# TheRealOrange/icer_compression

Hardware: AMD Instinct MI355X
Metric: Mpixels/s encode (bit-exact), 4096x4096 gray (higher is better)
Workload: dtype int16

## Files before the change

### icer_compression_amd/csrc/api.hip

```cpp
#include <hip/hip_runtime.h>

#include <algorithm>
#include <atomic>
#include <map>
#include <memory>
#include <mutex>
#include <thread>
#include <sched.h>
#include <time.h>
#include <stdarg.h>
#include <stdio.h>
#include <stdlib.h>
#include <string.h>
#include <string>
#include <vector>

#include "../../include/icer_hip.h"
#include "kernels.hpp"
#include "launch_plan.hpp"
#include "subband_gain.hpp"

using namespace icer;

namespace {
// ... 204 lines not shown
    DevBuf<uint32_t> sub_order, snap_valid;
    DevBuf<Snapshot> snaps;
    DevBuf<SubRecord> sub_recs;
    hipStream_t side_stream = nullptr;
    bool side_stream_borrowed = false;
    hipEvent_t fork[kMaxParts] = {}, join[kMaxParts] = {};
    hipStream_t half_stream = nullptr;
    hipEvent_t part_fork = nullptr, part_join = nullptr;
    hipEvent_t coef_ready = nullptr;
    hipStream_t io_stream = nullptr, copy_stream = nullptr;
    DevBuf<CoderTables> tables;
    DevBuf<uint16_t> in;
    DevBuf<uint8_t> in8;
    DevBuf<uint8_t> out;
    DevBuf<unsigned long long> sizes;
    DevBuf<int32_t> rcs;
    DevBuf<uint64_t> prof;
    DevBuf<unsigned long long> dist;
    DevBuf<uint32_t> fam_weight;
    DevBuf<uint32_t> fam_chan;
    DevBuf<unsigned long long> fam_ll_term;
    hipEvent_t energy_fork[kMaxParts] = {}, energy_join[kMaxParts] = {};
    int dist_frames = 0;
    DevBuf<unsigned long long> curve;
    DevBuf<uint32_t> curve_head;
    DevBuf<BudgetState> budget_state;

    DevBuf<uint64_t> roi_prio;
    DevBuf<uint64_t> roi_keys;
    DevBuf<uint32_t> roi_rank, roi_order;
    DevBuf<uint32_t> roi_bits;

    int *h_flag = nullptr;
    hipEvent_t done = nullptr;
    bool wg_available = true;
    bool sleepy_wait = false;
    struct Pending {
        bool active = false;
        EncodeCall call = {};
    } pend;

    bool timing = false;
    hipEvent_t ev[ICERX_NUM_STAGES + 1] = {};
    double ms[ICERX_NUM_STAGES] = {};
    uint64_t timed_calls = 0;
    bool ev_pending = false;

    int *dwt_ovf(int f0) const { return flags.p + (size_t)f0 * channels; }
    int *mean_ovf(int f0) const { return flags.p + (size_t)max_frames * channels + (size_t)f0 * channels; }
    int *skip(int f0) const { return flags.p + 2 * (size_t)max_frames * channels + f0; }
    int *bound_ovf() const { return flags.p + 2 * (size_t)max_frames * channels + max_frames; }
};

namespace {

struct ClearList {
    static constexpr int kMax = 10;
    uint32_t *p[kMax];
    uint32_t words[kMax];
    int n = 0;
    bool add(void *ptr, size_t bytes)
    {
        if (bytes && (n == kMax || bytes % 4 || bytes / 4 > UINT32_MAX)) return false;
        if (bytes) { p[n] = static_cast<uint32_t *>(ptr); words[n] = (uint32_t)(bytes / 4); n++; }
        return true;
    }
// ... 173 lines not shown
                       b.d_total, e->bound_ovf(), e->budget_state.p);
    hipLaunchKernelGGL(gather_ladder_kernel, dim3(n_units, b.n_frames), dim3(256), 0, c.stream, e->slots.p, e->plan.slot_bytes, e->units.p, n_units,
                       e->unit_bits.p, e->final_off.p, off_pitch, (uint32_t)b.n, c.d_out, c.out_stride, (uint32_t)b.n_frames);
    HIP_TRY(hipGetLastError());
    return 0;
}

int enqueue_part(icerx_encoder *e, const LaunchPlan &lp, int part, bool timed, const EncodeCall &c, bool clear_bound)
{
    const PartPlan &pp = lp.part[part];
    const int f0 = pp.f0, n_frames = pp.n_frames;
    const uint16_t *const d_frames = c.d_frames; uint8_t *const d_out = c.d_out; int32_t *const d_rcs = c.d_rcs;
    unsigned long long *const d_sizes = reinterpret_cast<unsigned long long *>(c.d_sizes);
    const size_t quota = c.quota, out_stride = c.out_stride;
    const hipStream_t st = c.stream; const Ladder *const ladder = c.ladder; const Target *const target = c.target; const Budget *const budget = c.budget;
    const Roi *const roi = c.roi;
    const bool energy = target || budget;
    const bool progressive = lp.progressive, use_wg = lp.use_wg, split = pp.split, hybrid = pp.hybrid;
    const size_t W = e->w, H = e->h, plane = W * H;
    const int C = e->channels, P = n_frames * C;
    const uint32_t n_units = (uint32_t)e->plan.units.size();
    int *dwt_ovf = e->dwt_ovf(f0), *mean_ovf = e->mean_ovf(f0), *skip = e->skip(f0), *bound_ovf = e->bound_ovf();
    int16_t *const coef = e->coef.p + (size_t)f0 * C * plane, *const tmp = e->tmp.p + (size_t)f0 * C * plane;
    unsigned long long *const sums = e->sums.p + (size_t)f0 * C;
    uint16_t *const means = e->means.p + (size_t)f0 * C;
    uint8_t *const sig = e->sig.p + (size_t)f0 * e->plan.sig_bytes;
    uint32_t *const sig_hist = e->sig_hist.p + (size_t)f0 * e->plan.n_families * 16;
    uint8_t *const route_buf = e->route.p + (size_t)f0 * n_units;
    uint32_t *const route_list = e->route_list.p + 2 * (size_t)f0 * n_units,        *const route_ctl = e->route_ctl.p + 4 * (size_t)part;
    uint8_t *const slots = e->slots.p + (size_t)f0 * e->plan.slot_bytes;
    uint32_t *const unit_bits = e->unit_bits.p + (size_t)f0 * n_units, *const done_bytes = e->done_bytes.p + (size_t)f0 * n_units;
    uint64_t *const final_off = e->final_off.p + (size_t)f0 * n_units;
    const size_t sub_entries = e->plan.sub_entries;
    if (split && (e->snaps.ensure((size_t)e->max_frames * sub_entries * kMaxSnaps) || e->snap_valid.ensure((size_t)e->max_frames * sub_entries * kMaxSnaps) ||
                  e->sub_recs.ensure((size_t)e->max_frames * sub_entries))) return ICER_FATAL_ERROR;
    {
        ClearList cl;
        const char *bad = nullptr;
        auto clear = [&](const char *what, void *ptr, size_t bytes) { if (!bad && !cl.add(ptr, bytes)) bad = what; };
        if (f0 == 0 && n_frames == e->max_frames && clear_bound) clear("frame flags", e->flags.p, e->flags.n * sizeof(int));
        else {
            clear("transform flags", dwt_ovf, (size_t)P * sizeof(int)); clear("mean flags", mean_ovf, (size_t)P * sizeof(int)); clear("skip flags", skip, (size_t)n_frames * sizeof(int));
            if (clear_bound) clear("slot bound flag", bound_ovf, sizeof(int));
        }
        clear("LL sums", sums, (size_t)P * sizeof(unsigned long long));
        if (progressive) clear("unit byte counts", done_bytes, (size_t)n_frames * n_units * 4);
        if (hybrid) { clear("chunk histograms", sig_hist, (size_t)n_frames * e->plan.n_families * 16 * sizeof(uint32_t)); clear("route list cursor", route_ctl, 4 * sizeof(uint32_t)); }
        if (split) { clear("snapshot flags", e->snap_valid.p, (size_t)n_frames * sub_entries * kMaxSnaps * sizeof(uint32_t)); clear("sub-range records", e->sub_recs.p, (size_t)n_frames * sub_entries * sizeof(SubRecord)); }
        if (bad) { set_error("enqueue: the clear kernel cannot take the %s range (%d ranges queued)", bad, cl.n); return ICER_FATAL_ERROR; }
        launch_clears(cl, st);
    }
    if (timed && e->timing) HIP_TRY(hipEventRecord(e->ev[0], st));

    size_t cw = W, ch = H;
    launch_dwt(e, d_frames, n_frames, st, e->sample_bits, dwt_ovf, &cw, &ch, coef, tmp);
    if (timed && e->timing) HIP_TRY(hipEventRecord(e->ev[1], st));

    const uint32_t llw = (uint32_t)cw, llh = (uint32_t)ch;
    unsigned sum_blocks = (llw * llh + 255) / 256;
    if (sum_blocks > 64) sum_blocks = 64;
    hipLaunchKernelGGL(ll_sum_kernel, dim3(sum_blocks, P), dim3(256), 0, st, reinterpret_cast<const uint16_t *>(coef),
                       plane, (uint32_t)W, llw, llh, sums, e->sample_bits == 8 ? 0xFFu : 0xFFFFu);
    hipLaunchKernelGGL(ll_mean_kernel, dim3((P + 63) / 64), dim3(64), 0, st, sums, (uint32_t)P, llw * llh,
                       means, mean_ovf, e->sample_bits);
    hipLaunchKernelGGL(frame_status_kernel, dim3((n_frames + 63) / 64), dim3(64), 0, st, dwt_ovf, mean_ovf, C, n_frames, skip);
    hipLaunchKernelGGL(finalize_ll_kernel, dim3((llw + 63u) / 64u, (llh + 3u) / 4u, P), dim3(256), 0, st,
                       reinterpret_cast<uint16_t *>(coef), plane, (uint32_t)W, llw, llh, means, skip, C, e->sample_bits);
    if (timed && e->timing) HIP_TRY(hipEventRecord(e->ev[2], st));
    if (e->coef_ready && f0 == 0) HIP_TRY(hipEventRecord(e->coef_ready, st));

    const int n_planes = e->sample_bits == 8 ? kPlanes8 : kPlanes;
    const size_t ev_frame_bytes = (size_t)n_planes * e->plan.sig_bytes * 64u;
    {
        hipLaunchKernelGGL(family_events_kernel, dim3((unsigned)(e->plan.sig_blocks.size() / 2), n_frames), dim3(256), 0, st,
                           reinterpret_cast<const uint16_t *>(coef), plane, (uint32_t)W, C, e->units.p, e->sig_blocks.p, skip, sig,
                           e->plan.sig_bytes, hybrid ? sig_hist : nullptr, e->plan.n_families,
                           use_wg ? nullptr : e->events.p + (size_t)f0 * ev_frame_bytes, ev_frame_bytes, (uint32_t)n_planes);
    }
    const uint8_t *route = nullptr;
    if (hybrid) {
        hipLaunchKernelGGL(route_units_kernel, dim3((unsigned)((n_units + 255) / 256), n_frames), dim3(256), 0, st, e->units.p, n_units, sig_hist, e->plan.n_families,
                           pp.route_percent, 16u, route_buf, route_list, route_ctl, kNoSplitPercent, (uint32_t)n_frames * n_units, kListHeavyMin);
        route = route_buf;
        HIP_TRY(hipEventRecord(e->fork[part], st));
        HIP_TRY(hipStreamWaitEvent(e->side_stream, e->fork[part], 0));
#define ICER_LAUNCH_LIST(I, NS)                                                                                                          \
        hipLaunchKernelGGL((code_units_list_kernel<I>), dim3(pp.list_grid), dim3(64 * NS::kWgWaves), sizeof(NS::Shared), e->side_stream, \
                           reinterpret_cast<const uint16_t *>(coef), plane, (uint32_t)W, (uint32_t)H, C, e->units.p, n_units,     \
                           e->tables.p, means, skip, slots, e->plan.slot_bytes, unit_bits, sig,                     \
                           e->plan.sig_bytes, route_list, route_ctl, e->prof.p ? e->prof.p + kProfWgsOffset : nullptr, (uint32_t)n_frames * n_units)
        if (pp.list == ListKernel::One) ICER_LAUNCH_LIST(WgOne, wg1); else if (pp.list == ListKernel::Four) ICER_LAUNCH_LIST(WgFour, wg4); else ICER_LAUNCH_LIST(WgSmall, wgs);
#undef ICER_LAUNCH_LIST
        HIP_TRY(hipEventRecord(e->join[part], e->side_stream));
    }
    const uint32_t tgt_planes = (uint32_t)n_planes;
    unsigned long long *const dist = energy ? e->dist.p + (size_t)f0 * e->plan.n_families * (tgt_planes + 1u) : nullptr;
    auto launch_energy = [&](hipStream_t es) -> int {
        HIP_TRY(hipMemsetAsync(dist, 0, (size_t)n_frames * e->plan.n_families * (tgt_planes + 1u) * sizeof(unsigned long long), es));
        hipLaunchKernelGGL(family_energy_kernel, dim3((unsigned)(e->plan.sig_blocks.size() / 2), n_frames), dim3(64 * kEnergyWaves), 0, es,
                           reinterpret_cast<const uint16_t *>(coef), plane, (uint32_t)W, C, e->units.p, e->sig_blocks.p, dist, e->plan.n_families, tgt_planes);
// ... 40 lines not shown
                           sig, e->plan.sig_bytes)
        if (pp.window == WindowKernel::Four) ICER_LAUNCH_WG(WgFour, wg4); else ICER_LAUNCH_WG(WgFull, wg);
#undef ICER_LAUNCH_WG
    }
    if (timed && e->timing) HIP_TRY(hipEventRecord(e->ev[3], st));

    if (energy) {
        if (e->side_stream) HIP_TRY(hipStreamWaitEvent(st, e->energy_join[part], 0));
        else if (launch_energy(st)) return ICER_FATAL_ERROR;
    }
    if (budget) {
        const size_t curve_pitch = (size_t)n_units + 1u;
        hipLaunchKernelGGL(curve_kernel, dim3(n_frames), dim3(64), 0, st, unit_bits, n_units, (uint64_t)quota, skip, e->units.p, dist, e->fam_weight.p,
                           e->plan.n_families, tgt_planes, e->fam_ll_term.p, e->fam_chan.p, means, C, e->curve.p + (size_t)f0 * curve_pitch,
                           e->curve.p + ((size_t)e->max_frames + f0) * curve_pitch, e->curve_head.p + (size_t)f0 * kCurveHeadWords);
        if (lp.n_parts == 1 && enqueue_budget_tail(e, c)) return ICER_FATAL_ERROR;
    } else if (target) {
        const size_t off_pitch = (size_t)e->max_frames * n_units;
        hipLaunchKernelGGL(scan_target_kernel, dim3(n_frames, target->n), dim3(64), 0, st, unit_bits, e->final_order.p, n_units, target->thresholds,
                           (uint64_t)quota, skip, final_off, off_pitch, d_sizes, d_rcs, (uint32_t)target->pitch, e->units.p, bound_ovf, dist,
                           e->fam_weight.p, e->plan.n_families, tgt_planes, e->fam_ll_term.p, e->fam_chan.p, means, C, target->d_reached + f0, target->d_dist + f0, target->d_equiv + f0);
        hipLaunchKernelGGL(gather_ladder_kernel, dim3(n_units, n_frames), dim3(256), 0, st, slots, e->plan.slot_bytes,
                           e->units.p, n_units, unit_bits, final_off, off_pitch, (uint32_t)target->n, d_out, out_stride, (uint32_t)target->pitch);
    } else if (roi) {
        const size_t off_pitch = (size_t)e->max_frames * n_units;
        uint32_t *const rank = e->roi_rank.p + (size_t)f0 * n_units, *const order = e->roi_order.p + (size_t)f0 * n_units;
        hipLaunchKernelGGL(roi_rank_kernel, dim3(n_frames), dim3(64 * kRoiWaves), 0, st, e->units.p, n_units, e->roi_prio.p, roi->d_rois + 4 * (size_t)f0,
                           roi->shift, (uint32_t)W, (uint32_t)H, e->roi_keys.p + (size_t)f0 * n_units, rank, order, roi->d_foreground + f0);
        hipLaunchKernelGGL(scan_roi_kernel, dim3(n_frames, roi->n), dim3(64), 0, st, unit_bits, e->final_order.p, n_units, roi->quotas, skip, rank, order,
                           e->roi_bits.p + (size_t)f0 * n_units, final_off, off_pitch, d_sizes, d_rcs, roi->d_kept + f0, (uint32_t)roi->pitch, e->units.p, bound_ovf);
        hipLaunchKernelGGL(gather_ladder_kernel, dim3(n_units, n_frames), dim3(256), 0, st, slots, e->plan.slot_bytes,
                           e->units.p, n_units, unit_bits, final_off, off_pitch, (uint32_t)roi->n, d_out, out_stride, (uint32_t)roi->pitch);
    } else if (!ladder || ladder->n == 1) {
        hipLaunchKernelGGL(scan_kernel, dim3(n_frames), dim3(64), 0, st, unit_bits, e->final_order.p, n_units,
                           (uint64_t)quota, skip, final_off, d_sizes, d_rcs, e->units.p, bound_ovf);
        hipLaunchKernelGGL(gather_kernel, dim3(n_units, n_frames), dim3(256), 0, st, slots, e->plan.slot_bytes,
                           e->units.p, n_units, unit_bits, final_off, d_out, out_stride);
    } else {
        const size_t off_pitch = (size_t)e->max_frames * n_units;
        hipLaunchKernelGGL(scan_ladder_kernel, dim3(n_frames, ladder->n), dim3(64), 0, st, unit_bits, e->final_order.p, n_units,
                           ladder->quotas, skip, final_off, off_pitch, d_sizes, d_rcs, (uint32_t)ladder->pitch, e->units.p, bound_ovf);
        hipLaunchKernelGGL(gather_ladder_kernel, dim3(n_units, n_frames), dim3(256), 0, st, slots, e->plan.slot_bytes,
                           e->units.p, n_units, unit_bits, final_off, off_pitch, (uint32_t)ladder->n, d_out, out_stride, (uint32_t)ladder->pitch);
    }
    if (timed && e->timing) {
        HIP_TRY(hipEventRecord(e->ev[4], st));
        e->ev_pending = true;
    }
    HIP_TRY(hipGetLastError());
    return 0;
}

int enqueue(icerx_encoder *e, const EncodeCall &c, bool overlap_ok)
{
    const hipStream_t st = c.stream;
    const CoderState cs{e->wg_available, e->wg_once, e->half_stream != nullptr};
    const LaunchPlan &lp = e->last_plan = plan_launch(launch_shape(e), e->tuning, cs, c.n_frames, c.quota, overlap_ok, c.roi != nullptr);
    if (lp.n_parts == 1) return enqueue_part(e, lp, 0, true, c, true);
    HIP_TRY(hipMemsetAsync(e->bound_ovf(), 0, sizeof(int), st));
    HIP_TRY(hipEventRecord(e->part_fork, st));
    HIP_TRY(hipStreamWaitEvent(e->half_stream, e->part_fork, 0));
    if (e->timing) { HIP_TRY(hipEventRecord(e->ev[0], st)); HIP_TRY(hipEventRecord(e->ev[1], st)); HIP_TRY(hipEventRecord(e->ev[2], st)); }
    for (int k = 0; k < lp.n_parts; k++) {
        EncodeCall pc = c.frames(lp.part[k].f0, lp.part[k].n_frames, (size_t)e->channels * e->w * e->h);
        pc.stream = (k & 1) ? e->half_stream : st;
        if (int rc = enqueue_part(e, lp, k, false, pc, false)) return rc;
    }
    HIP_TRY(hipEventRecord(e->part_join, e->half_stream));
// ... 68 lines not shown
#define CREATE_TRY(expr) do { hipError_t e_ = (expr); if (e_ != hipSuccess) { set_error("%s failed: %s (%s:%d)", #expr, hipGetErrorString(e_), __FILE__, __LINE__); icerx_encoder_destroy(e); return ICER_FATAL_ERROR; } } while (0)
    CREATE_TRY(hipSetDevice(device));
    const size_t P = (size_t)max_frames * channels, plane = w * h, n_units = e->plan.units.size();
    if (e->coef.ensure(P * plane) || e->tmp.ensure(P * plane) || e->sums.ensure(P) || e->means.ensure(P) ||
        e->flags.ensure(2 * P + 2 * max_frames + 1) || e->unit_bits.ensure((size_t)max_frames * n_units) ||
        e->done_bytes.ensure((size_t)max_frames * n_units) || e->route.ensure((size_t)max_frames * n_units) || e->route_list.ensure(2 * (size_t)max_frames * n_units) || e->route_ctl.ensure(4 * kMaxParts) || e->sig.ensure((size_t)max_frames * e->plan.sig_bytes + 64) || e->sig_hist.ensure((size_t)max_frames * e->plan.n_families * 16 + 16) ||
        e->final_off.ensure((size_t)max_frames * n_units) || e->tables.ensure(1) || e->sizes.ensure(max_frames) ||
        e->rcs.ensure(max_frames)) {
        icerx_encoder_destroy(e);
        return ICER_FATAL_ERROR;
    }
    if (e->tuning.coder != 2 && e->events.ensure((size_t)max_frames * (size_t)(sample_bits == 8 ? kPlanes8 : kPlanes) * e->plan.sig_bytes * 64u + 64)) {
        icerx_encoder_destroy(e);
        return ICER_FATAL_ERROR;
    }
    CREATE_TRY(hipMemcpy(e->tables.p, &g_tables, sizeof g_tables, hipMemcpyHostToDevice));
    if (hipFuncSetAttribute(reinterpret_cast<const void *>(code_units_wg_kernel<WgFull>), hipFuncAttributeMaxDynamicSharedMemorySize, (int)sizeof(wg::Shared)) != hipSuccess ||
        hipFuncSetAttribute(reinterpret_cast<const void *>(code_units_wg_kernel<WgFour>), hipFuncAttributeMaxDynamicSharedMemorySize, (int)sizeof(wg4::Shared)) != hipSuccess ||
        hipFuncSetAttribute(reinterpret_cast<const void *>(code_units_list_kernel<WgSmall>), hipFuncAttributeMaxDynamicSharedMemorySize, (int)sizeof(wgs::Shared)) != hipSuccess ||
        hipFuncSetAttribute(reinterpret_cast<const void *>(code_units_list_kernel<WgOne>), hipFuncAttributeMaxDynamicSharedMemorySize, (int)sizeof(wg1::Shared)) != hipSuccess ||
        hipFuncSetAttribute(reinterpret_cast<const void *>(code_units_list_kernel<WgFour>), hipFuncAttributeMaxDynamicSharedMemorySize, (int)sizeof(wg4::Shared)) != hipSuccess ||
        create_side_stream(&e->side_stream) != hipSuccess ||
        create_part_events(e) != hipSuccess) {
        (void)hipGetLastError();
        e->wg_available = false;
        if (e->tuning.coder == 2) { set_error("ICER_HIP_CODER=wg, but this device does not grant the workgroup coder its LDS block"); icerx_encoder_destroy(e); return ICER_FATAL_ERROR; }
        fprintf(stderr, "libicer_hip: the workgroup coder is not available on this device; the wave pipeline codes everything\n");
    }
#ifdef ICER_PHASE_TIMERS
    if (e->prof.ensure(kProfWords)) { icerx_encoder_destroy(e); return ICER_FATAL_ERROR; }
    CREATE_TRY(hipMemset(e->prof.p, 0, kProfWords * sizeof(uint64_t)));
#endif
    for (auto &ev : e->ev) CREATE_TRY(hipEventCreate(&ev));
    CREATE_TRY(hipHostMalloc((void **)&e->h_flag, (2 + kMaxParts) * sizeof(int), hipHostMallocDefault));
    CREATE_TRY(hipEventCreateWithFlags(&e->done, hipEventDisableTiming));
#undef CREATE_TRY
    *out = e;
    return 0;
}

void icerx_encoder_destroy(icerx_encoder *e)
{
    if (!e) return;
    (void)hipSetDevice(e->device);
    e->coef.release(); e->tmp.release(); e->sums.release(); e->means.release(); e->flags.release();
    e->units.release(); e->work_order.release(); e->final_order.release(); e->unit_bits.release(); e->done_bytes.release(); e->sig.release(); e->events.release(); e->sig_hist.release(); e->sig_blocks.release(); e->route.release(); e->route_list.release(); e->route_ctl.release();
    e->final_off.release(); e->slots.release(); e->tables.release(); e->in.release(); e->in8.release(); e->out.release();
    e->sizes.release(); e->rcs.release(); e->prof.release();
    e->subs.release(); e->sub_order.release(); e->snap_valid.release(); e->snaps.release(); e->sub_recs.release();
    e->dist.release(); e->fam_weight.release(); e->fam_chan.release(); e->fam_ll_term.release();
    e->curve.release(); e->curve_head.release(); e->budget_state.release();
    e->roi_prio.release(); e->roi_keys.release(); e->roi_rank.release(); e->roi_order.release(); e->roi_bits.release();
    for (auto &ev : e->energy_fork) if (ev) (void)hipEventDestroy(ev);
    for (auto &ev : e->energy_join) if (ev) (void)hipEventDestroy(ev);
    for (auto &ev : e->ev) if (ev) (void)hipEventDestroy(ev);
    if (e->done) (void)hipEventDestroy(e->done);
    for (auto &ev : e->fork) if (ev) (void)hipEventDestroy(ev);
    for (auto &ev : e->join) if (ev) (void)hipEventDestroy(ev);
    if (e->part_fork) (void)hipEventDestroy(e->part_fork);
    if (e->part_join) (void)hipEventDestroy(e->part_join);
    if (e->half_stream) (void)hipStreamDestroy(e->half_stream);
    if (e->side_stream && !e->side_stream_borrowed) (void)hipStreamDestroy(e->side_stream);
    if (e->coef_ready) (void)hipEventDestroy(e->coef_ready);
    if (e->io_stream) (void)hipStreamDestroy(e->io_stream);
    if (e->copy_stream) (void)hipStreamDestroy(e->copy_stream);
    if (e->h_flag) (void)hipHostFree(e->h_flag);
    delete e;
// ... 9 lines not shown
    std::vector<uint32_t> bits((size_t)n_frames * n_units);
    if (!n_units || hipMemcpy(bits.data(), e->unit_bits.p, bits.size() * sizeof(uint32_t), hipMemcpyDeviceToHost) != hipSuccess) return;
    int shown = 0;
    for (size_t i = 0; i < bits.size() && shown < 4; i++) {
        if (bits[i] != kUnitFailed) continue;
        const size_t frame = i / n_units, ui = i % n_units;
        const UnitDesc &u = e->plan.units[ui];
        uint32_t dbg[kFailWords] = {0};
        if (u.cap_words >= kFailWords)
            (void)hipMemcpy(dbg, e->slots.p + frame * e->plan.slot_bytes + u.slot_off + kHeaderBytes, sizeof dbg, hipMemcpyDeviceToHost);
        fprintf(stderr, "libicer_hip: time-out in frame %zu unit %zu (chan %u level %u subband %u lsb %u seg %u, %u x %u)", frame, ui,
                (unsigned)u.chan, (unsigned)u.level, (unsigned)u.subband, (unsigned)u.lsb, (unsigned)u.seg, (unsigned)u.w, (unsigned)u.h);
        if (dbg[0] == kFailMagic)
            fprintf(stderr, ": wave %u gave up at coder_core.hpp:%u; chunks %u, done pixel/count/compact/merge %u/%u/%u/%u, ring alloc/popped "
                    "%u/%u, hold seq/ack %u/%u, generation %u (last exact %u), bitpos %u, flushed words %u, drain_exit %u",
                    dbg[1] >> 16, dbg[1] & 0xFFFFu, dbg[2], dbg[3], dbg[4], dbg[5], dbg[6], dbg[7], dbg[8], dbg[9], dbg[10], dbg[11],
                    dbg[12], dbg[13], dbg[14], dbg[15]);
        fprintf(stderr, "\n");
        shown++;
    }
}

size_t row_stride(const icerx_encoder *e, size_t quota) { return std::min(quota, e->plan.slot_bytes) + 4; }
bool stride_admissible(const icerx_encoder *e, size_t out_stride, size_t quota) { return out_stride >= quota || out_stride >= e->plan.slot_bytes; }

int encode_begin(icerx_encoder *e, const EncodeCall &c, int *flag, hipEvent_t done)
{
    if (upload_units(e, c.quota, c.stream)) return ICER_FATAL_ERROR;
    if (e->slots.ensure((size_t)e->max_frames * e->plan.slot_bytes)) return ICER_FATAL_ERROR;
    if (!stride_admissible(e, c.out_stride, c.quota)) {
        set_error("icerx_encode_device: out_stride %zu smaller than the byte quota %zu", c.out_stride, c.quota);
        return ICER_INVALID_INPUT;
    }
    if (enqueue(e, c, c.overlap_ok && flag == e->h_flag)) return ICER_FATAL_ERROR;
    HIP_TRY(hipMemcpyAsync(flag, e->bound_ovf(), sizeof(int), hipMemcpyDeviceToHost, c.stream));
    for (int k = 0; k < e->last_plan.n_parts; k++)
        if (e->last_plan.part[k].hybrid) HIP_TRY(hipMemcpyAsync(flag + 1 + k, e->route_ctl.p + 4 * k, sizeof(int), hipMemcpyDeviceToHost, c.stream));
    HIP_TRY(hipEventRecord(done, c.stream));
    return 0;
}

static int wait_event(hipEvent_t ev, bool sleepy)
{
    for (uint32_t polls = 0;; polls++) {
        const hipError_t q = hipEventQuery(ev);
        if (q == hipSuccess) return 0;
        if (q != hipErrorNotReady) { set_error("hipEventQuery failed: %s", hipGetErrorString(q)); return ICER_FATAL_ERROR; }
        if (sleepy && polls > 64u) { const struct timespec ts = {0, 50000}; nanosleep(&ts, nullptr); }
        else cpu_relax();
    }
}

static int encode_verdict(icerx_encoder *e, int n_frames, const int *flag)
{
    const int ovf = flag[0];
    if (!ovf) {
        bool routed = false;
        for (int k = 0; k < e->last_plan.n_parts; k++) if (e->last_plan.part[k].hybrid) { routed = true; e->n_routed_units += (uint64_t)(uint32_t)flag[1 + k]; }
        if (routed) e->n_routed_launches++;
        return 0;
    }
    if (ovf & 2) {
        report_timeouts(e, n_frames);
        e->n_timeouts++; g_stats[0]++;
        if (e->wg_once || !e->wg_available) {
            e->wg_once = false;
            set_error(e->wg_available ? "a coding unit timed out in the workgroup-window coder"
                                      : "a coding unit timed out and the barrier-only coder is not available on this device");
            return ICER_FATAL_ERROR;
        }
// ... 977 lines not shown
```

### icer_compression_amd/csrc/dwt_tile.hpp

```cpp
#pragma once
#include <stdint.h>

#if defined(__HIPCC__)
#define DWT_HD __host__ __device__ __forceinline__
#else
#define DWT_HD static inline
#endif
#include "icer_tables.hpp"

#if defined(__HIPCC__)
#define DWT_UNROLL _Pragma("unroll")
#else
#define DWT_UNROLL
#endif

namespace icer {

constexpr int kTileKX = 64, kTileKY = 16;
constexpr int kWinW = 2 * kTileKX + 8, kWinH = 2 * kTileKY + 8;
constexpr int kWinPX = kWinW / 2, kWinPY = kWinH / 2;
constexpr int kTileThreads = 256;

struct DwtTileShared {
    union {
// ... 13 lines not shown
    const int16_t *src;
    uint32_t src_stride;
    int cw, ch;
    int16_t *coef;
    uint32_t coef_stride;
    int16_t *ll;
    uint32_t ll_stride;
    FilterTaps f;
    int32_t lim;
    int sm;
};

DWT_HD int16_t to_coder_word(int16_t v, int sm)
{
    if (sm == 16) {
        const uint16_t mask = (uint16_t)(v >> 15);
        return (int16_t)((((uint16_t)v + mask) ^ mask) | ((uint16_t)v & 0x8000u));
    }
    if (sm == 8) {
        const int8_t v8 = (int8_t)v;
        const uint8_t m8 = (uint8_t)(v8 >> 7);
        const uint8_t w8 = (uint8_t)((((uint8_t)v8 + m8) ^ m8) | ((uint8_t)v8 & 0x80u));
        return (int16_t)(uint16_t)(((w8 & 0x80u) << 8) | (w8 & 0x7Fu));
    }
    return v;
}

DWT_HD int tile_x0(int tx) { return 2 * tx * kTileKX - 4; }
DWT_HD int tile_y0(int ty) { return 2 * ty * kTileKY - 4; }

DWT_HD void dwt_tile_load(DwtTileShared &sh, const DwtStageArgs &a, int tx, int ty, int t)
{
    const int x0 = tile_x0(tx), y0 = tile_y0(ty);
    const bool words = ((a.src_stride & 1u) == 0u) && ((reinterpret_cast<uintptr_t>(a.src) & 3u) == 0u);
    for (int i = t; i < kWinH * kWinPX; i += kTileThreads) {
        const int r = i / kWinPX, p = i - r * kWinPX;
        const int gx = x0 + 2 * p, gy = y0 + r;
        int16_t v0 = 0, v1 = 0;
        if (gy >= 0 && gy < a.ch && gx + 1 >= 0 && gx < a.cw) {
            const int16_t *q = a.src + (size_t)gy * a.src_stride + gx;
            if (words && gx >= 0 && gx + 1 < a.cw) {
                const uint32_t w = *reinterpret_cast<const uint32_t *>(q);
                v0 = (int16_t)(w & 0xFFFFu); v1 = (int16_t)(w >> 16);
            } else {
                if (gx >= 0) v0 = q[0];
                if (gx + 1 < a.cw) v1 = q[1];
            }
        }
        sh.win[r][2 * p] = v0; sh.win[r][2 * p + 1] = v1;
    }
}

DWT_HD bool dwt_pair_step1(int32_t a, int32_t b, int n, int k, int32_t lim, int16_t *low, int16_t *dif)
{
    const int nh = n >> 1;
    bool ovf = false;
    if (k < nh) {
        const int32_t v = (a + b) >> 1, d = a - b;
        ovf = v < -lim - 1 || v > lim || d < -lim - 1 || d > lim;
        *low = (int16_t)v; *dif = (int16_t)d;
    } else { *low = (int16_t)a; *dif = 0; }
    return ovf;
}

template <class Lo, class Di>
DWT_HD bool dwt_pair_step2(const Lo &LO, const Di &DI, int n, int k, int am1, int a0, int a1, int be, int32_t lim, int16_t *high)
{
    const int nl = (n + 1) >> 1, nh = n >> 1;
    const bool odd = (n & 1) != 0;
    const auto clampi = [nl](int j) { return j < 0 ? 0 : (j > nl - 1 ? nl - 1 : j); };
    const int32_t l0 = LO(clampi(k - 2)), l1 = LO(clampi(k - 1)), l2 = LO(k), l3 = LO(clampi(k + 1));
    const int32_t r_km1 = (int16_t)(l0 - l1), r_k = (int16_t)(l1 - l2), r_kp1 = (int16_t)(l2 - l3);
    const int32_t dk = DI(k);
    const int32_t dn = (k + 1 < nh) ? (int32_t)DI(k + 1) : 0;
    int32_t sub;
    if (k == 0) sub = r_kp1 >> 2;
    else if (k == 1 && am1 != 0) {
        const int32_t x = (odd && nl == 3) ? 0 : dk;
        sub = (2 * r_k + 3 * r_kp1 - 2 * x + 4) >> 3;
    } else if (!odd && k == nh - 1) sub = r_k >> 2;
    else {
        const int32_t rm = (k >= 2) ? r_km1 : 1;
// ... 222 lines not shown
```

### icer_compression_amd/csrc/kernels.hpp

```cpp
#pragma once
#include <hip/hip_runtime.h>

#include "assemble_core.hpp"
#include "assemble_ladder.hpp"
#include "roi_core.hpp"
#include "coder_core.hpp"
#include "distortion_core.hpp"
#include "budget_core.hpp"
#include "coder_wg.hpp"
#include "coder_wg_small.hpp"
#include "dwt_tile.hpp"
#include "events.hpp"
#include "plan.hpp"

namespace icer {

__global__ void __launch_bounds__(kTileThreads)
dwt_tile_kernel(DwtStageArgs a, size_t src_plane, size_t coef_plane, size_t ll_plane, int *__restrict__ ovf)
{
    __shared__ union { DwtTileShared gen; DwtFastShared fast; } u;
    a.src += blockIdx.z * src_plane;
    a.coef += blockIdx.z * coef_plane;
    a.ll += blockIdx.z * ll_plane;
    const int tx = blockIdx.x, ty = blockIdx.y, t = threadIdx.x;
// ... 26 lines not shown
              unsigned long long *__restrict__ sums, uint32_t mask)
{
    const uint16_t *p = coef + blockIdx.y * plane;
    const uint32_t n = llw * llh;
    unsigned long long acc = 0;
    for (uint32_t i = blockIdx.x * 256 + threadIdx.x; i < n; i += gridDim.x * 256) {
        const uint32_t r = i / llw, c = i - r * llw;
        acc += p[(size_t)r * stride + c] & mask;
    }
    for (int o = 32; o > 0; o >>= 1) acc += __shfl_down(acc, o);
    if ((threadIdx.x & 63) == 0 && acc) atomicAdd(&sums[blockIdx.y], acc);
}

__global__ void ll_mean_kernel(const unsigned long long *__restrict__ sums, uint32_t n_planes, uint32_t ll_count,
                               uint16_t *__restrict__ means, int *__restrict__ mean_ovf, int sample_bits)
{
    const uint32_t p = blockIdx.x * blockDim.x + threadIdx.x;
    if (p >= n_planes) return;
    const uint16_t m = sample_bits == 8 ? (uint16_t)(uint8_t)(sums[p] / ll_count) : (uint16_t)(sums[p] / ll_count);
    means[p] = m;
    mean_ovf[p] = m > (sample_bits == 8 ? 127 : 32767) ? 1 : 0;
}

__global__ void __launch_bounds__(256)
finalize_ll_kernel(uint16_t *__restrict__ coef, size_t plane, uint32_t w, uint32_t llw, uint32_t llh,
                   const uint16_t *__restrict__ means, const int *__restrict__ frame_skip, int channels, int sample_bits)
{
    const uint32_t c = blockIdx.x * 64 + (threadIdx.x & 63), r = blockIdx.y * 4 + (threadIdx.x >> 6);
    if (c >= llw || r >= llh) return;
    if (frame_skip[blockIdx.z / channels]) return;
    uint16_t *q = coef + blockIdx.z * plane + (size_t)r * w + c;
    const int16_t v = (int16_t)((int16_t)*q - (int16_t)means[blockIdx.z]);
    *q = (uint16_t)to_coder_word(v, sample_bits);
}

struct SplitLaunch {
    const SubDesc *subs = nullptr;
    const uint32_t *launch = nullptr;
    uint32_t n_subs = 0;
    uint32_t entries = 0;
    Snapshot *snaps = nullptr;
    uint32_t *snap_valid = nullptr;
    SubRecord *recs = nullptr;
};

constexpr uint8_t kRoutePipeline = 0, kRouteWindows = 1, kRouteNoSplit = 2;

template <int WAVES, int OCC, int LDS_PAD>
__global__ void __launch_bounds__(64 * WAVES, OCC)
code_units_kernel(const uint16_t *__restrict__ coef, size_t plane, uint32_t img_w, uint32_t img_h, int channels,
                  const UnitDesc *__restrict__ units, const uint32_t *__restrict__ work_order, uint32_t n_units,
                  const CoderTables *__restrict__ tables, const uint16_t *__restrict__ means,
                  const int *__restrict__ frame_skip, uint8_t *__restrict__ slots,
                  size_t slot_frame_stride, uint32_t *__restrict__ unit_bits, uint64_t *__restrict__ timers,
                  uint32_t *__restrict__ done_bytes, uint64_t early_quota, const uint8_t *__restrict__ route, SplitLaunch sp, uint32_t n_frames_1d,
                  const uint8_t *__restrict__ ev, size_t ev_frame_stride, const uint8_t *__restrict__ sig, size_t sig_frame_stride,
                  uint32_t fail_inject)
{
    __shared__ CoderShared s;
    if constexpr (LDS_PAD > 0) {
        __shared__ uint32_t lds_pad[LDS_PAD / 4];
        if (early_quota == ~0ull) lds_pad[threadIdx.x] = 1u;
    }
    uint32_t frame = blockIdx.y, lpos = blockIdx.x;
    if (gridDim.y == 1u && n_frames_1d > 1u) {
        position_major(blockIdx.x, n_units + sp.n_subs, n_frames_1d, &frame, &lpos);
// ... 453 lines not shown
                       size_t slot_frame_stride, uint32_t *__restrict__ unit_bits,
                       const uint8_t *__restrict__ sig, size_t sig_frame_stride,
                       const uint32_t *__restrict__ list, uint32_t *__restrict__ list_ctl, uint64_t *__restrict__ timers, uint32_t list_cap)
{
    extern __shared__ __attribute__((aligned(16))) unsigned char wg_lds[];
    typename I::Shared &s = *reinterpret_cast<typename I::Shared *>(wg_lds);
    __shared__ uint32_t next_entry;
    wg_shared_tables<I>(s, tables);
    const WgLaunch L{coef, plane, img_w, img_h, channels, units, n_units, means, frame_skip, slots, slot_frame_stride, unit_bits, timers,
                     nullptr, 0ull, sig, sig_frame_stride};
    const uint32_t count = list_ctl[0], n_heavy = list_ctl[2];
    for (;;) {
        __syncthreads();
        if (threadIdx.x == 0) next_entry = atomicAdd(&list_ctl[1], 1u);
        __syncthreads();
        const uint32_t at = next_entry;
        if (at >= count) break;
        const uint32_t e = at < n_heavy ? list[list_cap + at] : list[at - n_heavy];
#ifdef ICER_PHASE_TIMERS
        const uint64_t t_start = wall_clock64();
#endif
        wg_code_one_unit<I>(s, L, e / n_units, e % n_units);
#ifdef ICER_PHASE_TIMERS
        if (timers && threadIdx.x == 0 && at < (uint32_t)kListTrace && e < n_units) {
            const UnitDesc &ud = units[e];
            uint64_t *tr = timers + 9 * 32 + 4 * at;
            tr[0] = t_start; tr[1] = wall_clock64(); tr[2] = blockIdx.x | ((uint64_t)e << 32);
            tr[3] = (uint64_t)ud.lsb | ((uint64_t)ud.level << 8) | ((uint64_t)ud.subband << 16) | ((uint64_t)ud.seg << 24) | ((uint64_t)((ud.w * ud.h + 63u) / 64u) << 32);
        }
#endif
    }
}

__global__ void __launch_bounds__(64)
scan_kernel(const uint32_t *__restrict__ unit_bits, const uint32_t *__restrict__ final_order, uint32_t n_units,
            uint64_t quota, const int *__restrict__ frame_skip, uint64_t *__restrict__ final_off,
            unsigned long long *__restrict__ sizes, int32_t *__restrict__ rcs, const UnitDesc *__restrict__ units,
            int *__restrict__ bound_overflow)
{
    const uint32_t frame = blockIdx.x;
    uint64_t *foff = final_off + (size_t)frame * n_units;
    if (frame_skip[frame]) {
        for (uint32_t i = threadIdx.x; i < n_units; i += 64) foff[i] = ~0ull;
        if (threadIdx.x == 0) { sizes[frame] = 0; rcs[frame] = kIntegerOverflow; }
        return;
    }
    const uint32_t *bits = unit_bits + (size_t)frame * n_units;
    {
        int failed = 0;
        for (uint32_t i = threadIdx.x; i < n_units; i += 64) failed |= bits[i] == kUnitFailed;
        if (__ballot(failed)) {
            for (uint32_t i = threadIdx.x; i < n_units; i += 64) foff[i] = ~0ull;
            if (threadIdx.x == 0) { sizes[frame] = 0; rcs[frame] = kFatalError; atomicOr(bound_overflow, 2); }
            return;
        }
    }
    uint32_t kept;
    uint64_t used;
    const int rc = scan_frame_wave(bits, final_order, n_units, quota, foff, &kept, &used);
    if (kept < n_units && threadIdx.x == 0 && bits[kept] == kUnitTooBig && units[kept].cap_is_bound)
        atomicOr(bound_overflow, 1);
    if (threadIdx.x == 0) { sizes[frame] = used; rcs[frame] = rc; }
}

__global__ void __launch_bounds__(256)
gather_kernel(const uint8_t *__restrict__ slots, size_t slot_frame_stride, const UnitDesc *__restrict__ units,
              uint32_t n_units, const uint32_t *__restrict__ unit_bits, const uint64_t *__restrict__ final_off,
              uint8_t *__restrict__ out, size_t out_stride)
{
    const uint32_t frame = blockIdx.y, ui = blockIdx.x;
    const uint64_t off = final_off[(size_t)frame * n_units + ui];
    if (off == ~0ull) return;
    const uint32_t len = kHeaderBytes + ((unit_bits[(size_t)frame * n_units + ui] + 7u) >> 3);
    const uint8_t *src = slots + (size_t)frame * slot_frame_stride + units[ui].slot_off;
    uint8_t *dst = out + (size_t)frame * out_stride + off;
    const uint32_t mis = (uint32_t)((4u - ((uintptr_t)dst & 3u)) & 3u);
    const uint32_t head = mis < len ? mis : len;
    if (threadIdx.x < head) dst[threadIdx.x] = src[threadIdx.x];
    const uint32_t body_words = (len - head) >> 2;
    const uint32_t *sw = reinterpret_cast<const uint32_t *>(src);
    uint32_t *dw = reinterpret_cast<uint32_t *>(dst + head);
    const uint32_t shift = head * 8;
    for (uint32_t i = threadIdx.x; i < body_words; i += 256) {
        const uint32_t lo = sw[i];
        uint32_t v = lo;
        if (shift) v = (lo >> shift) | (sw[i + 1] << (32 - shift));
        dw[i] = v;
    }
    const uint32_t done = head + body_words * 4;
    if (threadIdx.x < len - done) dst[done + threadIdx.x] = src[done + threadIdx.x];
}


__global__ void __launch_bounds__(64)
scan_ladder_kernel(const uint32_t *__restrict__ unit_bits, const uint32_t *__restrict__ final_order, uint32_t n_units,
// ... 156 lines not shown
```

Baseline: 3407.

## Fuse LL mean stages, parallelize scan, write verdict via mapped memory, batch DWT loads

For small LL bands, one block-per-plane kernel now replaces the four-kernel sum/mean/status/finalize sequence, and the LL-sums clear is dropped. The one-wave scan kernel becomes a 256-thread block scan with a cut search. The verdict words are written straight into mapped coherent host memory instead of being fetched with extra device-to-host memcpys. The DWT tile load is restructured to issue all loads before the LDS stores. This trims launch and copy overhead but adds a system-scope write, whose visibility ordering and bit-exactness carry risk.

```diff
diff --git a/icer_compression_amd/csrc/api.hip b/icer_compression_amd/csrc/api.hip
--- a/icer_compression_amd/csrc/api.hip
+++ b/icer_compression_amd/csrc/api.hip
@@ -260,6 +260,9 @@
     DevBuf<uint32_t> roi_bits;
 
     int *h_flag = nullptr;
+    int *d_flag = nullptr;
+    bool verdict_wanted = false;
+    bool verdict_written = false;
     hipEvent_t done = nullptr;
     bool wg_available = true;
     bool sleepy_wait = false;
@@ -499,6 +502,9 @@
     uint32_t *const unit_bits = e->unit_bits.p + (size_t)f0 * n_units, *const done_bytes = e->done_bytes.p + (size_t)f0 * n_units;
     uint64_t *const final_off = e->final_off.p + (size_t)f0 * n_units;
     const size_t sub_entries = e->plan.sub_entries;
+    size_t ll_w = W, ll_h = H;
+    for (int s = 0; s < e->stages; s++) { ll_w = (ll_w + 1) / 2; ll_h = (ll_h + 1) / 2; }
+    const bool ll_fused = P <= (int)kLlFusedMaxPlanes && ll_w * ll_h <= kLlFusedMaxSamples;
     if (split && (e->snaps.ensure((size_t)e->max_frames * sub_entries * kMaxSnaps) || e->snap_valid.ensure((size_t)e->max_frames * sub_entries * kMaxSnaps) ||
                   e->sub_recs.ensure((size_t)e->max_frames * sub_entries))) return ICER_FATAL_ERROR;
     {
@@ -510,7 +516,7 @@
             clear("transform flags", dwt_ovf, (size_t)P * sizeof(int)); clear("mean flags", mean_ovf, (size_t)P * sizeof(int)); clear("skip flags", skip, (size_t)n_frames * sizeof(int));
             if (clear_bound) clear("slot bound flag", bound_ovf, sizeof(int));
         }
-        clear("LL sums", sums, (size_t)P * sizeof(unsigned long long));
+        if (!ll_fused) clear("LL sums", sums, (size_t)P * sizeof(unsigned long long));
         if (progressive) clear("unit byte counts", done_bytes, (size_t)n_frames * n_units * 4);
         if (hybrid) { clear("chunk histograms", sig_hist, (size_t)n_frames * e->plan.n_families * 16 * sizeof(uint32_t)); clear("route list cursor", route_ctl, 4 * sizeof(uint32_t)); }
         if (split) { clear("snapshot flags", e->snap_valid.p, (size_t)n_frames * sub_entries * kMaxSnaps * sizeof(uint32_t)); clear("sub-range records", e->sub_recs.p, (size_t)n_frames * sub_entries * sizeof(SubRecord)); }
@@ -524,15 +530,21 @@
     if (timed && e->timing) HIP_TRY(hipEventRecord(e->ev[1], st));
 
     const uint32_t llw = (uint32_t)cw, llh = (uint32_t)ch;
-    unsigned sum_blocks = (llw * llh + 255) / 256;
-    if (sum_blocks > 64) sum_blocks = 64;
-    hipLaunchKernelGGL(ll_sum_kernel, dim3(sum_blocks, P), dim3(256), 0, st, reinterpret_cast<const uint16_t *>(coef),
-                       plane, (uint32_t)W, llw, llh, sums, e->sample_bits == 8 ? 0xFFu : 0xFFFFu);
-    hipLaunchKernelGGL(ll_mean_kernel, dim3((P + 63) / 64), dim3(64), 0, st, sums, (uint32_t)P, llw * llh,
-                       means, mean_ovf, e->sample_bits);
-    hipLaunchKernelGGL(frame_status_kernel, dim3((n_frames + 63) / 64), dim3(64), 0, st, dwt_ovf, mean_ovf, C, n_frames, skip);
-    hipLaunchKernelGGL(finalize_ll_kernel, dim3((llw + 63u) / 64u, (llh + 3u) / 4u, P), dim3(256), 0, st,
-                       reinterpret_cast<uint16_t *>(coef), plane, (uint32_t)W, llw, llh, means, skip, C, e->sample_bits);
+    const uint32_t ll_mask = e->sample_bits == 8 ? 0xFFu : 0xFFFFu;
+    if (ll_fused) {
+        hipLaunchKernelGGL(ll_fused_kernel, dim3(P), dim3(kLlFusedThreads), 0, st, reinterpret_cast<uint16_t *>(coef), plane, (uint32_t)W, llw, llh,
+                           ll_mask, C, e->sample_bits, dwt_ovf, means, mean_ovf, skip);
+    } else {
+        unsigned sum_blocks = (llw * llh + 255) / 256;
+        if (sum_blocks > 64) sum_blocks = 64;
+        hipLaunchKernelGGL(ll_sum_kernel, dim3(sum_blocks, P), dim3(256), 0, st, reinterpret_cast<const uint16_t *>(coef),
+                           plane, (uint32_t)W, llw, llh, sums, ll_mask);
+        hipLaunchKernelGGL(ll_mean_kernel, dim3((P + 63) / 64), dim3(64), 0, st, sums, (uint32_t)P, llw * llh,
+                           means, mean_ovf, e->sample_bits);
+        hipLaunchKernelGGL(frame_status_kernel, dim3((n_frames + 63) / 64), dim3(64), 0, st, dwt_ovf, mean_ovf, C, n_frames, skip);
+        hipLaunchKernelGGL(finalize_ll_kernel, dim3((llw + 63u) / 64u, (llh + 3u) / 4u, P), dim3(256), 0, st,
+                           reinterpret_cast<uint16_t *>(coef), plane, (uint32_t)W, llw, llh, means, skip, C, e->sample_bits);
+    }
     if (timed && e->timing) HIP_TRY(hipEventRecord(e->ev[2], st));
     if (e->coef_ready && f0 == 0) HIP_TRY(hipEventRecord(e->coef_ready, st));
 
@@ -639,8 +651,13 @@
         hipLaunchKernelGGL(gather_ladder_kernel, dim3(n_units, n_frames), dim3(256), 0, st, slots, e->plan.slot_bytes,
                            e->units.p, n_units, unit_bits, final_off, off_pitch, (uint32_t)roi->n, d_out, out_stride, (uint32_t)roi->pitch);
     } else if (!ladder || ladder->n == 1) {
-        hipLaunchKernelGGL(scan_kernel, dim3(n_frames), dim3(64), 0, st, unit_bits, e->final_order.p, n_units,
-                           (uint64_t)quota, skip, final_off, d_sizes, d_rcs, e->units.p, bound_ovf);
+        VerdictWords verdict;
+        if (e->verdict_wanted && lp.n_parts == 1 && n_frames == 1) {
+            verdict.host = e->d_flag; verdict.route_ctl = hybrid ? route_ctl : nullptr;
+            e->verdict_written = true;
+        }
+        hipLaunchKernelGGL(scan_kernel, dim3(n_frames), dim3(kScanThreads), 0, st, unit_bits, e->final_order.p, n_units,
+                           (uint64_t)quota, skip, final_off, d_sizes, d_rcs, e->units.p, bound_ovf, verdict);
         hipLaunchKernelGGL(gather_kernel, dim3(n_units, n_frames), dim3(256), 0, st, slots, e->plan.slot_bytes,
                            e->units.p, n_units, unit_bits, final_off, d_out, out_stride);
     } else {
@@ -775,7 +792,14 @@
     CREATE_TRY(hipMemset(e->prof.p, 0, kProfWords * sizeof(uint64_t)));
 #endif
     for (auto &ev : e->ev) CREATE_TRY(hipEventCreate(&ev));
-    CREATE_TRY(hipHostMalloc((void **)&e->h_flag, (2 + kMaxParts) * sizeof(int), hipHostMallocDefault));
+    const char *const verdict_mode = getenv("ICER_HIP_VERDICT");
+    if ((verdict_mode && !strcmp(verdict_mode, "copy")) ||
+        hipHostMalloc((void **)&e->h_flag, (2 + kMaxParts) * sizeof(int), hipHostMallocMapped | hipHostMallocCoherent) != hipSuccess ||
+        hipHostGetDevicePointer((void **)&e->d_flag, e->h_flag, 0) != hipSuccess) {
+        (void)hipGetLastError();
+        e->d_flag = nullptr;
+        if (!e->h_flag) CREATE_TRY(hipHostMalloc((void **)&e->h_flag, (2 + kMaxParts) * sizeof(int), hipHostMallocDefault));
+    }
     CREATE_TRY(hipEventCreateWithFlags(&e->done, hipEventDisableTiming));
 #undef CREATE_TRY
     *out = e;
@@ -851,10 +875,14 @@
         set_error("icerx_encode_device: out_stride %zu smaller than the byte quota %zu", c.out_stride, c.quota);
         return ICER_INVALID_INPUT;
     }
+    e->verdict_wanted = flag == e->h_flag && e->d_flag;
+    e->verdict_written = false;
     if (enqueue(e, c, c.overlap_ok && flag == e->h_flag)) return ICER_FATAL_ERROR;
-    HIP_TRY(hipMemcpyAsync(flag, e->bound_ovf(), sizeof(int), hipMemcpyDeviceToHost, c.stream));
-    for (int k = 0; k < e->last_plan.n_parts; k++)
-        if (e->last_plan.part[k].hybrid) HIP_TRY(hipMemcpyAsync(flag + 1 + k, e->route_ctl.p + 4 * k, sizeof(int), hipMemcpyDeviceToHost, c.stream));
+    if (!e->verdict_written) {
+        HIP_TRY(hipMemcpyAsync(flag, e->bound_ovf(), sizeof(int), hipMemcpyDeviceToHost, c.stream));
+        for (int k = 0; k < e->last_plan.n_parts; k++)
+            if (e->last_plan.part[k].hybrid) HIP_TRY(hipMemcpyAsync(flag + 1 + k, e->route_ctl.p + 4 * k, sizeof(int), hipMemcpyDeviceToHost, c.stream));
+    }
     HIP_TRY(hipEventRecord(done, c.stream));
     return 0;
 }
diff --git a/icer_compression_amd/csrc/dwt_tile.hpp b/icer_compression_amd/csrc/dwt_tile.hpp
--- a/icer_compression_amd/csrc/dwt_tile.hpp
+++ b/icer_compression_amd/csrc/dwt_tile.hpp
@@ -69,22 +69,26 @@
 DWT_HD void dwt_tile_load(DwtTileShared &sh, const DwtStageArgs &a, int tx, int ty, int t)
 {
     const int x0 = tile_x0(tx), y0 = tile_y0(ty);
-    const bool words = ((a.src_stride & 1u) == 0u) && ((reinterpret_cast<uintptr_t>(a.src) & 3u) == 0u);
-    for (int i = t; i < kWinH * kWinPX; i += kTileThreads) {
+    constexpr int kIters = (kWinH * kWinPX + kTileThreads - 1) / kTileThreads;
+    int16_t v0[kIters], v1[kIters];
+    DWT_UNROLL
+    for (int k = 0; k < kIters; k++) {
+        const int i = t + k * kTileThreads;
         const int r = i / kWinPX, p = i - r * kWinPX;
         const int gx = x0 + 2 * p, gy = y0 + r;
-        int16_t v0 = 0, v1 = 0;
-        if (gy >= 0 && gy < a.ch && gx + 1 >= 0 && gx < a.cw) {
-            const int16_t *q = a.src + (size_t)gy * a.src_stride + gx;
-            if (words && gx >= 0 && gx + 1 < a.cw) {
-                const uint32_t w = *reinterpret_cast<const uint32_t *>(q);
-                v0 = (int16_t)(w & 0xFFFFu); v1 = (int16_t)(w >> 16);
-            } else {
-                if (gx >= 0) v0 = q[0];
-                if (gx + 1 < a.cw) v1 = q[1];
-            }
-        }
-        sh.win[r][2 * p] = v0; sh.win[r][2 * p + 1] = v1;
+        const bool row_in = i < kWinH * kWinPX && gy >= 0 && gy < a.ch;
+        const bool in0 = row_in && gx >= 0 && gx < a.cw, in1 = row_in && gx + 1 >= 0 && gx + 1 < a.cw;
+        const size_t at0 = in0 ? (size_t)gy * a.src_stride + (size_t)gx : 0u, at1 = in1 ? (size_t)gy * a.src_stride + (size_t)(gx + 1) : 0u;
+        const int16_t s0 = a.src[at0], s1 = a.src[at1];
+        v0[k] = in0 ? s0 : (int16_t)0;
+        v1[k] = in1 ? s1 : (int16_t)0;
+    }
+    DWT_UNROLL
+    for (int k = 0; k < kIters; k++) {
+        const int i = t + k * kTileThreads;
+        if (i >= kWinH * kWinPX) break;
+        const int r = i / kWinPX, p = i - r * kWinPX;
+        sh.win[r][2 * p] = v0[k]; sh.win[r][2 * p + 1] = v1[k];
     }
 }
 
diff --git a/icer_compression_amd/csrc/kernels.hpp b/icer_compression_amd/csrc/kernels.hpp
--- a/icer_compression_amd/csrc/kernels.hpp
+++ b/icer_compression_amd/csrc/kernels.hpp
@@ -82,6 +82,66 @@
     uint16_t *q = coef + blockIdx.z * plane + (size_t)r * w + c;
     const int16_t v = (int16_t)((int16_t)*q - (int16_t)means[blockIdx.z]);
     *q = (uint16_t)to_coder_word(v, sample_bits);
+}
+
+constexpr uint32_t kLlFusedThreads = 1024, kLlFusedMaxSamples = 1u << 16, kLlFusedMaxPlanes = 4, kLlFusedBatch = 8;
+__global__ void __launch_bounds__(kLlFusedThreads)
+ll_fused_kernel(uint16_t *__restrict__ coef, size_t plane, uint32_t stride, uint32_t llw, uint32_t llh, uint32_t mask, int channels,
+                int sample_bits, const int *__restrict__ dwt_ovf, uint16_t *__restrict__ means, int *__restrict__ mean_ovf,
+                int *__restrict__ frame_skip)
+{
+    __shared__ unsigned long long wave_sum[kLlFusedThreads / 64];
+    const uint32_t p = blockIdx.x, frame = p / (uint32_t)channels, n = llw * llh;
+    int skip = 0;
+    uint16_t mean = 0;
+    for (uint32_t q = frame * (uint32_t)channels; q < (frame + 1u) * (uint32_t)channels; q++) {
+        const uint16_t *src = coef + q * plane;
+        unsigned long long acc = 0;
+        for (uint32_t base = threadIdx.x; base < n; base += kLlFusedBatch * kLlFusedThreads) {
+            uint32_t v[kLlFusedBatch];
+#pragma unroll
+            for (uint32_t k = 0; k < kLlFusedBatch; k++) {
+                const uint32_t i = base + k * kLlFusedThreads, ii = i < n ? i : 0u;
+                const uint32_t r = ii / llw, c = ii - r * llw;
+                const uint32_t x = src[(size_t)r * stride + c];
+                v[k] = i < n ? x & mask : 0u;
+            }
+#pragma unroll
+            for (uint32_t k = 0; k < kLlFusedBatch; k++) acc += v[k];
+        }
+        for (int o = 32; o > 0; o >>= 1) acc += __shfl_down(acc, o);
+        if ((threadIdx.x & 63) == 0) wave_sum[threadIdx.x >> 6] = acc;
+        __syncthreads();
+        unsigned long long sum = 0;
+        for (uint32_t w = 0; w < kLlFusedThreads / 64; w++) sum += wave_sum[w];
+        __syncthreads();
+        const uint16_t m = sample_bits == 8 ? (uint16_t)(uint8_t)(sum / n) : (uint16_t)(sum / n);
+        const int ovf = m > (sample_bits == 8 ? 127 : 32767) ? 1 : 0;
+        skip |= dwt_ovf[q] | ovf;
+        if (q == p) {
+            mean = m;
+            if (threadIdx.x == 0) { means[p] = m; mean_ovf[p] = ovf; }
+        }
+    }
+    if (threadIdx.x == 0 && p == frame * (uint32_t)channels) frame_skip[frame] = skip;
+    if (skip) return;
+    uint16_t *dst = coef + p * plane;
+    for (uint32_t base = threadIdx.x; base < n; base += kLlFusedBatch * kLlFusedThreads) {
+        uint16_t v[kLlFusedBatch];
+        size_t at[kLlFusedBatch];
+#pragma unroll
+        for (uint32_t k = 0; k < kLlFusedBatch; k++) {
+            const uint32_t i = base + k * kLlFusedThreads, ii = i < n ? i : 0u;
+            const uint32_t r = ii / llw, c = ii - r * llw;
+            at[k] = (size_t)r * stride + c;
+            v[k] = dst[at[k]];
+        }
+#pragma unroll
+        for (uint32_t k = 0; k < kLlFusedBatch; k++) {
+            if (base + k * kLlFusedThreads >= n) break;
+            dst[at[k]] = (uint16_t)to_coder_word((int16_t)((int16_t)v[k] - (int16_t)mean), sample_bits);
+        }
+    }
 }
 
 struct SplitLaunch {
@@ -601,35 +661,100 @@
     }
 }
 
-__global__ void __launch_bounds__(64)
+struct VerdictWords {
+    int *host = nullptr;
+    const uint32_t *route_ctl = nullptr;
+};
+
+constexpr uint32_t kScanThreads = 256;
+
+__device__ inline uint64_t scan_block_exclusive(uint64_t v, uint64_t *wave_tot, uint64_t *total)
+{
+    const uint32_t lane = threadIdx.x & 63u, wv = threadIdx.x >> 6;
+    uint64_t inc = v;
+    for (uint32_t o = 1; o < 64u; o <<= 1) {
+        const uint64_t t = __shfl_up((unsigned long long)inc, o);
+        if (lane >= o) inc += t;
+    }
+    if (lane == 63u) wave_tot[wv] = inc;
+    __syncthreads();
+    uint64_t base = 0, tot = 0;
+    for (uint32_t w = 0; w < kScanThreads / 64u; w++) {
+        const uint64_t x = wave_tot[w];
+        if (w < wv) base += x;
+        tot += x;
+    }
+    __syncthreads();
+    *total = tot;
+    return base + inc - v;
+}
+
+__global__ void __launch_bounds__(kScanThreads)
 scan_kernel(const uint32_t *__restrict__ unit_bits, const uint32_t *__restrict__ final_order, uint32_t n_units,
             uint64_t quota, const int *__restrict__ frame_skip, uint64_t *__restrict__ final_off,
             unsigned long long *__restrict__ sizes, int32_t *__restrict__ rcs, const UnitDesc *__restrict__ units,
-            int *__restrict__ bound_overflow)
-{
+            int *__restrict__ bound_overflow, VerdictWords verdict)
+{
+    __shared__ uint64_t wave_tot[kScanThreads / 64];
+    __shared__ uint32_t cut;
     const uint32_t frame = blockIdx.x;
     uint64_t *foff = final_off + (size_t)frame * n_units;
+    auto publish = [&]() {
+        if (!verdict.host) return;
+        __hip_atomic_store(&verdict.host[0], __hip_atomic_load(bound_overflow, __ATOMIC_RELAXED, __HIP_MEMORY_SCOPE_AGENT), __ATOMIC_RELAXED, __HIP_MEMORY_SCOPE_SYSTEM);
+        if (verdict.route_ctl) __hip_atomic_store(&verdict.host[1], (int)verdict.route_ctl[0], __ATOMIC_RELAXED, __HIP_MEMORY_SCOPE_SYSTEM);
+    };
     if (frame_skip[frame]) {
-        for (uint32_t i = threadIdx.x; i < n_units; i += 64) foff[i] = ~0ull;
-        if (threadIdx.x == 0) { sizes[frame] = 0; rcs[frame] = kIntegerOverflow; }
+        for (uint32_t i = threadIdx.x; i < n_units; i += kScanThreads) foff[i] = ~0ull;
+        if (threadIdx.x == 0) { sizes[frame] = 0; rcs[frame] = kIntegerOverflow; publish(); }
         return;
     }
     const uint32_t *bits = unit_bits + (size_t)frame * n_units;
-    {
-        int failed = 0;
-        for (uint32_t i = threadIdx.x; i < n_units; i += 64) failed |= bits[i] == kUnitFailed;
-        if (__ballot(failed)) {
-            for (uint32_t i = threadIdx.x; i < n_units; i += 64) foff[i] = ~0ull;
-            if (threadIdx.x == 0) { sizes[frame] = 0; rcs[frame] = kFatalError; atomicOr(bound_overflow, 2); }
-            return;
-        }
-    }
-    uint32_t kept;
-    uint64_t used;
-    const int rc = scan_frame_wave(bits, final_order, n_units, quota, foff, &kept, &used);
-    if (kept < n_units && threadIdx.x == 0 && bits[kept] == kUnitTooBig && units[kept].cap_is_bound)
-        atomicOr(bound_overflow, 1);
-    if (threadIdx.x == 0) { sizes[frame] = used; rcs[frame] = rc; }
+    const uint32_t per = (n_units + kScanThreads - 1u) / kScanThreads;
+    const uint32_t first = threadIdx.x * per < n_units ? threadIdx.x * per : n_units;
+    const uint32_t last = first + per < n_units ? first + per : n_units;
+    int failed = 0;
+    uint64_t mine = 0;
+    for (uint32_t u = first; u < last; u++) {
+        const uint32_t v = bits[u];
+        failed |= v == kUnitFailed;
+        mine += (uint64_t)kHeaderBytes + (((uint64_t)v + 7u) >> 3);
+    }
+    if (threadIdx.x == 0) cut = n_units;
+    if (__syncthreads_or(failed)) {
+        for (uint32_t i = threadIdx.x; i < n_units; i += kScanThreads) foff[i] = ~0ull;
+        if (threadIdx.x == 0) { sizes[frame] = 0; rcs[frame] = kFatalError; atomicOr(bound_overflow, 2); publish(); }
+        return;
+    }
+    uint64_t total;
+    uint64_t before = scan_block_exclusive(mine, wave_tot, &total);
+    for (uint32_t u = first; u < last; u++) {
+        const uint32_t v = bits[u];
+        if (v == kUnitTooBig || before + kHeaderBytes > quota || (v > 0u && (uint64_t)(v >> 3) + before + kHeaderBytes >= quota)) {
+            atomicMin(&cut, u);
+            break;
+        }
+        before += (uint64_t)kHeaderBytes + (((uint64_t)v + 7u) >> 3);
+    }
+    __syncthreads();
+    const uint32_t K = cut;
+    mine = 0;
+    for (uint32_t j = first; j < last; j++) {
+        const uint32_t u = final_order[j];
+        if (u < K) mine += (uint64_t)kHeaderBytes + (((uint64_t)bits[u] + 7u) >> 3);
+    }
+    uint64_t off = scan_block_exclusive(mine, wave_tot, &total);
+    for (uint32_t j = first; j < last; j++) {
+        const uint32_t u = final_order[j];
+        if (u < K) { foff[u] = off; off += (uint64_t)kHeaderBytes + (((uint64_t)bits[u] + 7u) >> 3); }
+        else foff[u] = ~0ull;
+    }
+    if (threadIdx.x == 0) {
+        if (K < n_units && bits[K] == kUnitTooBig && units[K].cap_is_bound) atomicOr(bound_overflow, 1);
+        sizes[frame] = total;
+        rcs[frame] = K < n_units ? kByteQuotaExceeded : kOk;
+        publish();
+    }
 }
 
 __global__ void __launch_bounds__(256)
```

Result: no change. 3432 (median of 6 runs) (+0.7%).
